# aws-neuron/neuronx-distributed

Measured on AMD Instinct MI355X. Metric: tokens/sec (whole node) Llama-2-7B training, TP=num_gpus, seq=4096, higher is better.
Workload: dtype bf16; 1 GPU; model=llama2-7b, global_batch=32, seq_len=4096, parallelism=tp1, zero1=True

## Files before the change

### neuronx_distributed_amd/models/gpt2.py

```python

from dataclasses import dataclass

import torch
import torch.nn as nn

from ..parallel.layers import (
    ColumnParallelLinear,
    RowParallelLinear,
    ParallelEmbedding,
)
from ..parallel.layer_norm import LayerNorm
from ..parallel.loss_functions import parallel_cross_entropy

torch.fx.wrap("parallel_cross_entropy")
from ..parallel import parallel_state as ps
from ..kernels.flash_attn import flash_attn_func


@dataclass
class GPT2Config:
    hidden_size: int = 768
    num_hidden_layers: int = 12
    num_attention_heads: int = 12
    vocab_size: int = 50304
# ... 48 lines not shown
        qkv = self.c_attn(x)
        q, k, v = qkv.chunk(3, dim=-1)
        q = q.reshape(B, S, self.n_local, self.head_dim).transpose(1, 2)
        k = k.reshape(B, S, self.n_local, self.head_dim).transpose(1, 2)
        v = v.reshape(B, S, self.n_local, self.head_dim).transpose(1, 2)
        if kv_cache is not None:
            k, v = kv_cache.update(k.contiguous(), v.contiguous(), pos_offset)
        out = flash_attn_func(q.contiguous(), k.contiguous(), v.contiguous(),
                              causal=True)
        out = out.transpose(1, 2).reshape(B, S, -1)
        return self.c_proj(out)


class GPT2MLP(nn.Module):
    def __init__(self, cfg: GPT2Config):
        super().__init__()
        self.c_fc = ColumnParallelLinear(
            cfg.hidden_size, 4 * cfg.hidden_size, bias=True,
            gather_output=False, init_method=_init(cfg.initializer_range))
        self.c_proj = RowParallelLinear(
            4 * cfg.hidden_size, cfg.hidden_size, bias=True,
            input_is_parallel=True, init_method=_init(cfg.initializer_range))

    def forward(self, x):
        return self.c_proj(torch.nn.functional.gelu(self.c_fc(x)))


class GPT2Block(nn.Module):
    def __init__(self, cfg: GPT2Config):
        super().__init__()
        self.ln_1 = LayerNorm(cfg.hidden_size, eps=cfg.layer_norm_epsilon)
        self.attn = GPT2Attention(cfg)
        self.ln_2 = LayerNorm(cfg.hidden_size, eps=cfg.layer_norm_epsilon)
        self.mlp = GPT2MLP(cfg)

    def forward(self, x, pos_offset=0, kv_cache=None):
        x = x + self.attn(self.ln_1(x), pos_offset, kv_cache)
        return x + self.mlp(self.ln_2(x))


class GPT2LMHeadModel(nn.Module):
    def __init__(self, cfg: GPT2Config):
        super().__init__()
        self.config = cfg
        self.wte = ParallelEmbedding(cfg.vocab_size, cfg.hidden_size,
                                     init_method=_init(cfg.initializer_range))
        self.wpe = nn.Embedding(cfg.max_position_embeddings, cfg.hidden_size)
        nn.init.normal_(self.wpe.weight, std=cfg.initializer_range)
        self.h = nn.ModuleList(GPT2Block(cfg)
                               for _ in range(cfg.num_hidden_layers))
        self.ln_f = LayerNorm(cfg.hidden_size, eps=cfg.layer_norm_epsilon)
        self.lm_head = ColumnParallelLinear(
            cfg.hidden_size, cfg.vocab_size, bias=False, gather_output=False,
            init_method=_init(cfg.initializer_range))

    def forward(self, input_ids, labels=None, pos_offset=0, kv_caches=None):
        B, S = input_ids.shape
        pos = torch.arange(pos_offset, pos_offset + S,
                           device=input_ids.device)
        x = self.wte(input_ids) + self.wpe(pos)
        for i, block in enumerate(self.h):
            kc = kv_caches[i] if kv_caches is not None else None
            x = block(x, pos_offset, kc)
        x = self.ln_f(x)
        logits = self.lm_head(x)
        if labels is None:
            return logits
        shift = labels[:, 1:].contiguous()
        loss = parallel_cross_entropy(logits[:, :-1, :].contiguous(), shift)
        return loss.sum() / (shift != -100).sum().clamp(min=1)
```

### neuronx_distributed_amd/models/gpt_neox.py

```python

from dataclasses import dataclass

import torch
import torch.nn as nn

from .. import ops
from ..kernels.flash_attn import flash_attn_func
from ..parallel import parallel_state as ps
from ..parallel.layer_norm import LayerNorm
from ..parallel.layers import (
    ColumnParallelLinear,
    ParallelEmbedding,
    RowParallelLinear,
)
from ..parallel.loss_functions import parallel_cross_entropy

torch.fx.wrap("parallel_cross_entropy")


@dataclass
class GPTNeoXConfig:
    hidden_size: int = 6144
    intermediate_size: int = 24576
    num_hidden_layers: int = 44
# ... 83 lines not shown
                              causal=True)
        out = out.transpose(1, 2).reshape(B, S, -1)
        return self.dense(out)


class GPTNeoXMLP(nn.Module):
    def __init__(self, cfg: GPTNeoXConfig):
        super().__init__()
        self.dense_h_to_4h = ColumnParallelLinear(
            cfg.hidden_size, cfg.intermediate_size, bias=True,
            gather_output=False, init_method=_init(cfg.initializer_range))
        self.dense_4h_to_h = RowParallelLinear(
            cfg.intermediate_size, cfg.hidden_size, bias=True,
            input_is_parallel=True, init_method=_init(cfg.initializer_range))

    def forward(self, x):
        return self.dense_4h_to_h(
            torch.nn.functional.gelu(self.dense_h_to_4h(x)))


class GPTNeoXLayer(nn.Module):
    def __init__(self, cfg: GPTNeoXConfig):
        super().__init__()
        self.use_parallel_residual = cfg.use_parallel_residual
        self.input_layernorm = LayerNorm(cfg.hidden_size,
                                         eps=cfg.layer_norm_epsilon)
        self.post_attention_layernorm = LayerNorm(cfg.hidden_size,
                                                  eps=cfg.layer_norm_epsilon)
        self.attention = GPTNeoXAttention(cfg)
        self.mlp = GPTNeoXMLP(cfg)

    def forward(self, x, cos, sin, pos_offset=0, kv_cache=None):
        attn_out = self.attention(self.input_layernorm(x), cos, sin,
                                  pos_offset, kv_cache)
        if self.use_parallel_residual:
            return x + attn_out + self.mlp(self.post_attention_layernorm(x))
        h = x + attn_out
        return h + self.mlp(self.post_attention_layernorm(h))


class GPTNeoXForCausalLM(nn.Module):
    def __init__(self, cfg: GPTNeoXConfig):
        super().__init__()
        self.config = cfg
        self.embed_in = ParallelEmbedding(
            cfg.vocab_size, cfg.hidden_size,
            init_method=_init(cfg.initializer_range))
        self.layers = nn.ModuleList(GPTNeoXLayer(cfg)
                                    for _ in range(cfg.num_hidden_layers))
        self.final_layer_norm = LayerNorm(cfg.hidden_size,
                                          eps=cfg.layer_norm_epsilon)
        self.embed_out = ColumnParallelLinear(
            cfg.hidden_size, cfg.vocab_size, bias=False, gather_output=False,
            init_method=_init(cfg.initializer_range))
        cos, sin = ops.precompute_rope_freqs(
            cfg.max_position_embeddings,
            max(2, 2 * (int(cfg.head_dim * cfg.rotary_pct) // 2)),
            cfg.rope_theta)
        self.register_buffer("rope_cos", cos, persistent=False)
        self.register_buffer("rope_sin", sin, persistent=False)

    def reset_parameters(self):
        cfg = self.config
        cos, sin = ops.precompute_rope_freqs(
            cfg.max_position_embeddings,
            max(2, 2 * (int(cfg.head_dim * cfg.rotary_pct) // 2)),
            cfg.rope_theta, device=self.rope_cos.device)
        with torch.no_grad():
            self.rope_cos.copy_(cos)
            self.rope_sin.copy_(sin)

    def forward(self, input_ids, labels=None, pos_offset=0, kv_caches=None):
        x = self.embed_in(input_ids)
        for i, layer in enumerate(self.layers):
            kc = kv_caches[i] if kv_caches is not None else None
            x = layer(x, self.rope_cos, self.rope_sin, pos_offset, kc)
        x = self.final_layer_norm(x)
        logits = self.embed_out(x)
        if labels is None:
            return logits
        shift = labels[:, 1:].contiguous()
        loss = parallel_cross_entropy(logits[:, :-1, :].contiguous(), shift)
        return loss.sum() / (shift != -100).sum().clamp(min=1)
```

### neuronx_distributed_amd/models/llama.py

```python

import math
import os
from dataclasses import dataclass, field
from typing import Optional

import torch
import torch.nn as nn

from .. import ops
from ..parallel import parallel_state as ps
from ..parallel.layers import (
    ColumnParallelLinear,
    RowParallelLinear,
    ParallelEmbedding,
)
from ..parallel.qkv_linear import GQAQKVColumnParallelLinear
from ..parallel.loss_functions import parallel_cross_entropy

torch.fx.wrap("parallel_cross_entropy")
from ..parallel.mappings import (
    scatter_to_sequence_parallel_region,
    gather_from_sequence_parallel_region,
)
from ..kernels.flash_attn import flash_attn_func
# ... 337 lines not shown
        if (not isinstance(hidden, torch.fx.Proxy)
                and not self.training and not torch.is_grad_enabled()
                and hidden.is_cuda and hidden.dtype == torch.bfloat16
                and not self.config.sequence_parallel_enabled
                and self.config.hidden_size % 8 == 0
                and ops.add_rmsnorm_available()
                and all(hasattr(l, "forward_fused")
                        for l in self.layers)):
            residual, delta = hidden, None
            for i, layer in enumerate(self.layers):
                kc = kv_caches[i] if kv_caches is not None else None
                residual, delta = layer.forward_fused(
                    residual, delta, self.rope_cos, self.rope_sin,
                    pos_offset, kc)
            _, hidden = ops.add_rmsnorm(residual, delta, self.norm.weight,
                                        self.norm.variance_epsilon)
            return hidden
        if fused_norm_train_ok(self.config, hidden, self.training) \
                and kv_caches is None \
                and all(hasattr(l, "forward_fused_train")
                        and not l._forward_hooks
                        and not l._forward_pre_hooks
                        for l in self.layers):
            residual, delta = hidden, None
            for layer in self.layers:
                residual, delta = layer.forward_fused_train(
                    residual, delta, self.rope_cos, self.rope_sin,
                    pos_offset)
            _, hidden = ops.add_rmsnorm_train(delta, residual,
                                              self.norm.weight,
                                              self.norm.variance_epsilon)
        else:
            for i, layer in enumerate(self.layers):
                kc = kv_caches[i] if kv_caches is not None else None
                hidden = layer(hidden, self.rope_cos, self.rope_sin,
                               pos_offset, kc)
            hidden = self.norm(hidden)
        if self.config.sequence_parallel_enabled:
            hidden = gather_from_sequence_parallel_region(
                hidden, seq_dim=0, to_model_parallel=True)
            hidden = hidden.transpose(0, 1)
        return hidden


class LlamaForCausalLM(nn.Module):
    supports_tensor_position = True

    def __init__(self, config: LlamaConfig):
        super().__init__()
        self.config = config
        self.model = LlamaModel(config)
        self.lm_head = ColumnParallelLinear(
            config.hidden_size, config.vocab_size, bias=False,
            gather_output=False,
            init_method=_init_method(config.initializer_range))
        if config.tie_word_embeddings:
            self.lm_head.weight = self.model.embed_tokens.weight

    def forward(self, input_ids, labels=None, pos_offset=0, kv_caches=None):
        hidden = self.model(input_ids, pos_offset, kv_caches)
        if labels is not None and self.config.loss_chunks > 0:
            from ..utils.chunked_loss import chunked_lm_loss

            return chunked_lm_loss(hidden, self.lm_head, labels,
                                   num_chunks=self.config.loss_chunks)
        logits = self.lm_head(hidden)
        if labels is None:
            return logits
        shift = labels[:, 1:].contiguous()
        loss = parallel_cross_entropy(logits[:, :-1, :].contiguous(), shift)
        valid = (shift != -100).sum().clamp(min=1)
        return loss.sum() / valid
```

### neuronx_distributed_amd/models/mixtral.py

```python

from dataclasses import dataclass
from typing import Optional

import os

import torch
import torch.nn as nn

from ..moe.expert_mlps import ExpertMLPs
from ..moe.loss_function import load_balancing_loss_func
from ..moe.model import MoE
from ..moe.routing import (GroupLimitedRouter, RouterSinkhorn, RouterTopK)
from ..moe.shared_experts import SharedExperts
from ..parallel.layers import ColumnParallelLinear, ParallelEmbedding
from ..parallel.loss_functions import parallel_cross_entropy
from ..parallel.mappings import (
    gather_from_sequence_parallel_region,
    scatter_to_sequence_parallel_region,
)
from .. import ops
from .llama import (LlamaAttention, LlamaMLP, RMSNorm, _init_method,
                    fused_norm_train_ok)

torch.fx.wrap("parallel_cross_entropy")
# ... 151 lines not shown
        cos, sin = ops.precompute_rope_freqs(
            self.config.max_position_embeddings, self.config.head_dim,
            self.config.rope_theta, device=self.rope_cos.device)
        with torch.no_grad():
            self.rope_cos.copy_(cos)
            self.rope_sin.copy_(sin)

    def forward(self, input_ids, pos_offset=0, kv_caches=None):
        hidden = self.embed_tokens(input_ids)
        if self.config.sequence_parallel_enabled:
            hidden = hidden.transpose(0, 1).contiguous()
            hidden = scatter_to_sequence_parallel_region(hidden, seq_dim=0)
        all_router_logits = []
        if fused_norm_train_ok(self.config, hidden, self.training) \
                and kv_caches is None \
                and all(hasattr(l, "forward_fused_train")
                        and not l._forward_hooks
                        and not l._forward_pre_hooks
                        for l in self.layers):
            residual, delta = hidden, None
            for layer in self.layers:
                residual, delta, router_logits = layer.forward_fused_train(
                    residual, delta, self.rope_cos, self.rope_sin,
                    pos_offset)
                if router_logits is not None:
                    all_router_logits.append(router_logits)
            _, hidden = ops.add_rmsnorm_train(delta, residual,
                                              self.norm.weight,
                                              self.norm.variance_epsilon)
        else:
            for i, layer in enumerate(self.layers):
                kc = kv_caches[i] if kv_caches is not None else None
                hidden, router_logits = layer(hidden, self.rope_cos,
                                              self.rope_sin, pos_offset, kc)
                if router_logits is not None:
                    all_router_logits.append(router_logits)
            hidden = self.norm(hidden)
        if self.config.sequence_parallel_enabled:
            hidden = gather_from_sequence_parallel_region(
                hidden, seq_dim=0, to_model_parallel=True)
            hidden = hidden.transpose(0, 1)
        return hidden, all_router_logits


class MixtralForCausalLM(nn.Module):
    supports_tensor_position = True

    def __init__(self, config: MixtralConfig):
        super().__init__()
        self.config = config
        self.model = MixtralModel(config)
        self.lm_head = ColumnParallelLinear(
            config.hidden_size, config.vocab_size, bias=False,
            gather_output=False,
            init_method=_init_method(config.initializer_range))
        if config.tie_word_embeddings:
            self.lm_head.weight = self.model.embed_tokens.weight

    def forward(self, input_ids, labels=None, pos_offset=0, kv_caches=None):
        hidden, router_logits = self.model(input_ids, pos_offset, kv_caches)
        logits = self.lm_head(hidden)
        if labels is None:
            return logits
        shift = labels[:, 1:].contiguous()
        loss = parallel_cross_entropy(logits[:, :-1, :].contiguous(),
                                      shift).sum() / \
            (shift != -100).sum().clamp(min=1)
        if router_logits and self.config.router_aux_loss_coef > 0:
            aux = load_balancing_loss_func(
                torch.cat(router_logits, dim=0),
                self.config.num_local_experts,
                self.config.num_experts_per_tok)
            loss = loss + self.config.router_aux_loss_coef * aux
        return loss
```

### neuronx_distributed_amd/ops/__init__.py

```python

import ctypes
import math
import os
from typing import Optional

import torch

_LIB = None
_LIB_ERR = None


def _load():
    global _LIB, _LIB_ERR
    if _LIB is not None or _LIB_ERR is not None:
        return _LIB
    from .build import LIB

    if not os.path.exists(LIB):
        _LIB_ERR = f"{LIB} not built — run neuronx_distributed_amd.ops.build"
        return None
    try:
        lib = ctypes.CDLL(LIB)
    except OSError as e:
        _LIB_ERR = str(e)
# ... 414 lines not shown
            dk = dk_pq
            dv = dv_pq
        return dq, dk, dv, None, None, None


def flash_attn(q, k, v, causal=True, softmax_scale=None, window=0):
    scale = softmax_scale or 1.0 / math.sqrt(q.shape[-1])
    return _FlashAttnFn.apply(q, k, v, causal, scale, window)


def flash_attn_window_available() -> bool:
    lib = _load()
    return lib is not None and hasattr(lib, "flash_attn_fwd_window")


def flash_attn_windowed(q, k, v, window: int, softmax_scale=None):
    lib = _require_lib()
    B, Hq, S, D = q.shape
    Hkv = k.shape[1]
    assert D == 128 and q.dtype == torch.bfloat16
    scale = softmax_scale or 1.0 / math.sqrt(D)
    q, k, v = q.contiguous(), k.contiguous(), v.contiguous()
    out = torch.empty_like(q)
    lse = torch.empty(B, Hq, S, dtype=torch.float32, device=q.device)
    lib.flash_attn_fwd_window(_ptr(q), _ptr(k), _ptr(v), _ptr(out),
                              _ptr(lse), ctypes.c_int(B), ctypes.c_int(Hq),
                              ctypes.c_int(Hkv), ctypes.c_int(S),
                              ctypes.c_float(scale), ctypes.c_int(window),
                              _stream())
    return out



def adamw_step(master: torch.Tensor, m: torch.Tensor, v: torch.Tensor,
               grad_bf16: torch.Tensor, param_bf16: torch.Tensor,
               clip: Optional[torch.Tensor], lr: float, beta1: float,
               beta2: float, eps: float, weight_decay: float, step: int):
    lib = _require_lib()
    n = master.numel()
    assert m.numel() == n and v.numel() == n and grad_bf16.numel() == n
    assert grad_bf16.dtype == torch.bfloat16 and param_bf16.dtype == torch.bfloat16
    inv_bc1 = 1.0 / (1.0 - beta1 ** step)
    inv_bc2 = 1.0 / (1.0 - beta2 ** step)
    lib.adamw_step(ctypes.c_long(n), _ptr(master), _ptr(m), _ptr(v),
                   _ptr(grad_bf16), _ptr(param_bf16),
                   _ptr(clip) if clip is not None else None,
                   ctypes.c_float(lr), ctypes.c_float(beta1),
                   ctypes.c_float(beta2), ctypes.c_float(eps),
                   ctypes.c_float(weight_decay), ctypes.c_float(inv_bc1),
                   ctypes.c_float(inv_bc2), _stream())



_MOE_MB = 16


def moe_decode_available() -> bool:
    lib = _load()
    return lib is not None and hasattr(lib, "moe_decode_glu")


def moe_decode_glu(hidden: torch.Tensor, gate_up_w: torch.Tensor,
                   down_w: torch.Tensor, expert_affinities: torch.Tensor,
                   expert_index: torch.Tensor) -> torch.Tensor:
    lib = _require_lib()
    T, H = hidden.shape
    E, _, twoI = gate_up_w.shape
    I = twoI // 2
    assert H % 64 == 0 and I % 64 == 0, (H, I)
    k = expert_index.shape[1]
    dev = hidden.device

    flat_e = expert_index.reshape(-1)
    order = torch.argsort(flat_e, stable=True)
    sorted_e = flat_e[order].to(torch.long)
    sorted_tok = (order // k).to(torch.int32)

    counts = torch.bincount(flat_e, minlength=E)
    blocks_per_e = (counts + _MOE_MB - 1) // _MOE_MB
    nb = int(blocks_per_e.sum().item())
    if nb == 0:
        return hidden.new_zeros(T, H)
    blockbase = torch.cumsum(torch.nn.functional.pad(blocks_per_e, (1, 0)),
                             0)
    countbase = torch.cumsum(torch.nn.functional.pad(counts, (1, 0)), 0)

    within = torch.arange(T * k, device=dev) - countbase[sorted_e]
    padded_idx = (blockbase[sorted_e] + within // _MOE_MB) * _MOE_MB + \
        within % _MOE_MB

    slot_token = torch.zeros(nb * _MOE_MB, dtype=torch.int32, device=dev)
    slot_token[padded_idx] = sorted_tok
    aff = torch.zeros(nb * _MOE_MB, dtype=torch.float32, device=dev)
    aff[padded_idx] = expert_affinities.float()[
        sorted_tok.long(), sorted_e]

    block_expert = torch.repeat_interleave(
        torch.arange(E, device=dev), blocks_per_e).to(torch.int32)
    bi = torch.arange(nb, device=dev)
    block_ord = bi - blockbase[block_expert.long()]
    block_len = torch.clamp(counts[block_expert.long()] -
                            _MOE_MB * block_ord, 0, _MOE_MB).to(torch.int32)

    act = torch.empty(nb * _MOE_MB, I, dtype=torch.bfloat16, device=dev)
    out = torch.zeros(T, H, dtype=torch.float32, device=dev)
    hidden = hidden.contiguous()
# ... 199 lines not shown
```

### neuronx_distributed_amd/optimizer/zero_redundancy_optimizer.py

```python

import math
import os
from typing import Dict, List

import torch
import torch.distributed as dist

from ..parallel import comm, parallel_state as ps
from ..parallel.utils import param_is_tensor_parallel, param_is_expert_parallel
from ..utils.logger import get_logger

logger = get_logger(__name__)

_DEFAULT_BUCKET_CAP_MB = 130


def _bucket_cap_bytes():
    return int(os.environ.get("ALL_GATHER_REDUCE_SCATTER_BUCKET_CAP_MB",
                              _DEFAULT_BUCKET_CAP_MB)) * 1024 * 1024


class _Bucket:

    def __init__(self, params: List[torch.nn.Parameter], group_info,
                 group_index: int, optimizer_dtype,
                 fp32_grad_acc: bool = False):
        self.params = params
        self.group_info = group_info
        self.group_index = group_index
        self.fp32_grad_acc = fp32_grad_acc
        world = group_info.size
        device = params[0].device
        dtype = params[0].dtype

        numel = sum(p.numel() for p in params)
        self.padded = int(math.ceil(numel / world) * world)
        self.flat_param = torch.zeros(self.padded, dtype=dtype, device=device)
        grad_dtype = torch.float32 if fp32_grad_acc else dtype
        self.flat_grad = torch.zeros(self.padded, dtype=grad_dtype,
                                     device=device)

        self.segments = []
        off = 0
        with torch.no_grad():
            for p in params:
                n = p.numel()
                self.flat_param[off:off + n].copy_(p.data.reshape(-1))
                new_data = self.flat_param[off:off + n].view(p.shape)
                p.data = new_data
                if fp32_grad_acc:
                    seg = self.flat_grad[off:off + n]

                    def _acc(param, _seg=seg):
                        if param.grad is not None:
                            _seg.add_(param.grad.detach().reshape(-1).float())
                            param.grad = None

                    p.register_post_accumulate_grad_hook(_acc)
                else:
                    p.grad = self.flat_grad[off:off + n].view(p.shape)
                self.segments.append((p, off, off + n))
# ... 122 lines not shown
                        cur, ginfo, gi, self.optimizer_dtype,
                        self.use_fp32_grad_acc))


    def _bucket_grad_scale(self, b) -> float:
        ep_size = ps._GROUPS["ep"].size if "ep" in ps._GROUPS else 1
        if ep_size > 1 and b.group_info.name == "edp":
            return 1.0 / (b.group_info.size * ep_size)
        return 1.0 / b.group_info.size

    @torch.no_grad()
    def _reduce_scatter_grads(self):
        works = []
        for b in self.buckets:
            world = b.group_info.size
            scale = self._bucket_grad_scale(b)
            if world == 1:
                if scale != 1.0:
                    b.flat_grad.mul_(scale)
                b.grad_shard = b.flat_grad
                continue
            b.flat_grad.mul_(scale)
            if comm._backend_is_gloo(b.group_info.group):
                dist.all_reduce(b.flat_grad, group=b.group_info.group)
                b.grad_shard.copy_(b.flat_grad[b.shard_lo:b.shard_hi])
            else:
                w = dist.reduce_scatter_tensor(b.grad_shard, b.flat_grad,
                                               group=b.group_info.group,
                                               async_op=True)
                works.append(w)
        for w in works:
            w.wait()

    @torch.no_grad()
    def _clip_grads(self, apply: bool = True):
        device = self.buckets[0].master.device
        sq = torch.zeros(1, dtype=torch.float32, device=device)
        for b in self.buckets:
            sq += b.local_sq_norm()
        comm.all_reduce(sq, group=self._sharding_group)
        for name in ("tp", "pp"):
            if name in ps._GROUPS and ps._GROUPS[name].size > 1:
                comm.all_reduce(sq, group=ps._GROUPS[name])
        total_norm = sq.sqrt()
        self._grad_norm = total_norm.squeeze()
        clip = torch.clamp(self.max_norm / (total_norm + 1e-6), max=1.0)
        if apply:
            for b in self.buckets:
                b.grad_shard.mul_(clip)
        return clip

    @torch.no_grad()
    def _all_gather_params(self, copy_master: bool = True):
        works = []
        for b in self.buckets:
            shard = b.flat_param[b.shard_lo:b.shard_hi]
            if copy_master:
                shard.copy_(b.master.to(b.flat_param.dtype))
            world = b.group_info.size
            if world == 1:
                continue
            if comm._backend_is_gloo(b.group_info.group):
                parts = list(b.flat_param.chunk(world))
                dist.all_gather(parts, shard.clone(), group=b.group_info.group)
            else:
                w = dist.all_gather_into_tensor(b.flat_param, shard.clone(),
                                                group=b.group_info.group,
                                                async_op=True)
                works.append(w)
        for w in works:
            w.wait()

    def _use_fused(self) -> bool:
        from .. import ops

        return (self.use_fused_kernel
                and not self.use_fp32_grad_acc
                and self.optimizer_class is torch.optim.AdamW
                and self.optimizer_dtype == torch.float32
                and self.buckets and self.buckets[0].master.is_cuda
                and ops.is_available())

    @torch.no_grad()
    def _fused_step(self, clip):
        from .. import ops

        self._step_count = getattr(self, "_step_count", 0) + 1
        for b in self.buckets:
            group = self.param_groups[b.group_index]
            if not hasattr(b, "fused_m"):
                b.fused_m = torch.zeros_like(b.master)
                b.fused_v = torch.zeros_like(b.master)
            beta1, beta2 = group.get("betas", (0.9, 0.999))
            ops.adamw_step(b.master, b.fused_m, b.fused_v, b.grad_shard,
                           b.flat_param[b.shard_lo:b.shard_hi], clip,
                           group.get("lr", 1e-3), beta1, beta2,
                           group.get("eps", 1e-8),
                           group.get("weight_decay", 0.0), self._step_count)

    @torch.no_grad()
    def step(self, closure=None):
        loss = None
        if closure is not None:
            with torch.enable_grad():
                loss = closure()

# ... 84 lines not shown
```

### neuronx_distributed_amd/parallel/layers.py

```python

import math
import os
from typing import Callable, Optional

import torch
import torch.nn as nn
import torch.nn.functional as F
import torch.distributed as dist

from . import comm
from . import parallel_state as ps
from .mappings import (
    copy_to_tensor_model_parallel_region,
    gather_from_tensor_model_parallel_region,
    reduce_from_tensor_model_parallel_region,
    reduce_scatter_to_sequence_parallel_region,
    gather_from_sequence_parallel_region,
    scatter_to_tensor_model_parallel_region,
)
from .random import get_rng_state_tracker
from .utils import (
    create_local_weight,
    divide,
    set_tensor_model_parallel_attributes,
# ... 71 lines not shown
                      + (weight.shape[0],),
                      dtype=input_.dtype, device=input_.device)
    for t in range(world):
        owner = (me - t) % world
        works = []
        if t < world - 1:
            ops_ = [dist.P2POp(dist.isend, cur, nxt, group=tp_info.group),
                    dist.P2POp(dist.irecv, recv_buf, prv,
                               group=tp_info.group)]
            works = dist.batch_isend_irecv(ops_)
        out[owner * S:(owner + 1) * S] = F.linear(cur, weight)
        for w in works:
            w.wait()
        if t < world - 1:
            nxt_recv = spare if cur is src else cur
            cur = recv_buf
            recv_buf = nxt_recv
    if bias is not None:
        out = out + bias
    return out


class _RPLOverlappedLinearRS(torch.autograd.Function):

    @staticmethod
    def forward(ctx, input_parallel, weight):
        tp_info = ps.get_group_info("tp")
        world = tp_info.size
        me = tp_info.rank_in_group(dist.get_rank())
        ranks = tp_info.ranks_of(dist.get_rank())
        ctx.save_for_backward(input_parallel, weight)
        x = input_parallel.contiguous()
        assert x.shape[0] % world == 0
        Sc = x.shape[0] // world
        handles = []
        chunks = []
        mine = None
        for c in range(world):
            y = F.linear(x[c * Sc:(c + 1) * Sc], weight)
            chunks.append(y)
            handles.append(dist.reduce(y, dst=ranks[c],
                                       group=tp_info.group, async_op=True))
            if c == me:
                mine = y
        for h in handles:
            h.wait()
        return mine.clone()

    @staticmethod
    def backward(ctx, grad_output):
        input_parallel, weight = ctx.saved_tensors
        tp_info = ps.get_group_info("tp")
        g = comm.all_gather(grad_output.contiguous(), dim=0, group=tp_info)
        grad_input = g.matmul(weight)
        go2d = g.reshape(-1, g.shape[-1])
        in2d = input_parallel.reshape(-1, input_parallel.shape[-1])
        grad_weight = go2d.t().matmul(in2d)
        return grad_input, grad_weight


def _fp8_forward_enabled() -> bool:
    return os.environ.get("NXDA_FP8_LINEAR", "0") == "1"


def _fp8_eligible(x: torch.Tensor, w: torch.Tensor) -> bool:
    return (x.is_cuda and x.dtype == torch.bfloat16
            and w.dtype == torch.bfloat16
            and x.shape[-1] % 16 == 0 and w.shape[0] % 16 == 0
            and w.shape[0] >= 2 * w.shape[1]
            and x.numel() // x.shape[-1] >= 2048)


def _fp8_quantized_weight(weight: torch.Tensor):
    from ..quantization.quantization_config import (QuantizationConfig,
                                                    QuantizedDtype)
    from ..quantization.quantization_utils import quantize_symmetric

    key = (weight.data_ptr(), weight._version)
    cache = getattr(weight, "_fp8_cache", None)
    if cache is None or cache[0] != key:
        cfg = QuantizationConfig(quantized_dtype=QuantizedDtype.F8E4M3,
                                 quantize_activation=True)
        with torch.no_grad():
            qw, ws = quantize_symmetric(weight.detach(), cfg)
        cache = (key, qw, ws)
        weight._fp8_cache = cache
    return cache[1], cache[2]


def _forward_gemm(total_input: torch.Tensor, weight: torch.Tensor, bias):
    if _fp8_forward_enabled() and _fp8_eligible(total_input, weight):
        from ..quantization.quantization_utils import fp8_scaled_linear

        qw, ws = _fp8_quantized_weight(weight)
        with torch.no_grad():
            out = fp8_scaled_linear(total_input, qw, ws, total_input.dtype)
        if bias is not None:
            out = out + bias
        return out
    return F.linear(total_input, weight, bias)


class LinearWithAsyncCommunication(torch.autograd.Function):

    @staticmethod
    def forward(ctx, input_, weight, bias, async_grad_allreduce,
                sequence_parallel_enabled, save_for_backward=True):
        ctx.use_bias = bias is not None
        ctx.async_grad_allreduce = async_grad_allreduce
        ctx.sequence_parallel_enabled = sequence_parallel_enabled
        ctx.compute_weight_gradient = weight.requires_grad

        if sequence_parallel_enabled:
            tp_info = ps.get_group_info("tp")
            if os.environ.get("NXDA_SP_OVERLAP", "0") == "1" and \
                    tp_info.size > 1 and not ps.is_aot_mode():
                output = _sp_overlapped_linear(input_, weight, bias, tp_info)
                if save_for_backward:
                    if ctx.compute_weight_gradient:
                        ctx.save_for_backward(input_, weight)
                    else:
                        ctx.save_for_backward(weight)
                return output
            total_input = comm.all_gather(input_, dim=0, group=tp_info)
        else:
            total_input = input_

        output = _forward_gemm(total_input, weight, bias)

        if save_for_backward:
            if ctx.compute_weight_gradient:
                ctx.save_for_backward(input_, weight)
            else:
                ctx.save_for_backward(weight)
        return output

    @staticmethod
    def backward(ctx, grad_output):
        if ctx.compute_weight_gradient:
            input_, weight = ctx.saved_tensors
        else:
            (weight,) = ctx.saved_tensors
            input_ = None

        tp_info = ps.get_group_info("tp")
        handle = None

        grad_output = grad_output.contiguous()
        grad_input = grad_output.matmul(weight)

        if ctx.sequence_parallel_enabled and ctx.compute_weight_gradient:
            total_input = comm.all_gather(input_, dim=0, group=tp_info)
        else:
            total_input = input_

        if ctx.sequence_parallel_enabled:
            world = tp_info.size
            if world > 1 and not ps.is_aot_mode():
                gi = grad_input.contiguous()
                sub_shape = (gi.shape[0] // world,) + tuple(gi.shape[1:])
                grad_input_out = torch.empty(sub_shape, dtype=gi.dtype,
                                             device=gi.device)
                if comm._backend_is_gloo(tp_info.group):
                    dist.all_reduce(gi, group=tp_info.group)
                    rank = tp_info.rank_in_group(dist.get_rank())
                    grad_input_out.copy_(gi[rank * sub_shape[0]:(rank + 1) * sub_shape[0]])
                else:
                    handle = dist.reduce_scatter_tensor(
                        grad_input_out, gi, group=tp_info.group, async_op=True)
                grad_input = grad_input_out
        elif ctx.async_grad_allreduce:
            handle = comm.all_reduce(grad_input, group=tp_info, async_op=True)

        grad_weight = grad_bias = None
        if ctx.compute_weight_gradient:
            go2d = grad_output.reshape(-1, grad_output.shape[-1])
            in2d = total_input.reshape(-1, total_input.shape[-1])
            grad_weight = go2d.t().matmul(in2d)
            if ctx.use_bias:
                grad_bias = go2d.sum(dim=0)
        elif ctx.use_bias:
            grad_bias = grad_output.reshape(-1, grad_output.shape[-1]).sum(dim=0)

        if handle is not None:
            handle.wait()
        return grad_input, grad_weight, grad_bias, None, None, None


def linear_with_async_allreduce(input_, weight, bias=None,
                                async_grad_allreduce=False,
                                sequence_parallel_enabled=False):
    from .. import ops as _ops

    if _ops.use_skinny_linear(input_, weight, sequence_parallel_enabled):
        flat = input_.reshape(-1, input_.shape[-1]).contiguous()
        out = _ops.skinny_linear(flat, weight)
        if bias is not None:
            out = out + bias
        return out.reshape(*input_.shape[:-1], weight.shape[0])
    args = cast_if_autocast_enabled(input_, weight, bias)
    with torch.amp.autocast("cuda", enabled=False):
        return LinearWithAsyncCommunication.apply(
            *args, async_grad_allreduce, sequence_parallel_enabled)


class BaseParallelLinear(nn.Module):
    def reset_parameters(self):
        spec = getattr(self, "_reset_spec", None)
        if spec is None:
            return
        out_f, in_f, per_part, pdim, stride, init_method, dtype = spec
        _initialize_affine_weight(self.weight, out_f, in_f, per_part,
                                  partition_dim=pdim, init_method=init_method,
                                  stride=stride, dtype=dtype)
        if getattr(self, "bias", None) is not None:
            with torch.no_grad():
                self.bias.zero_()

    def _init_weight(self, weight, init_method):
        if getattr(weight, "device", torch.device("cpu")).type == "meta":
            return
        with get_rng_state_tracker().fork():
            init_method(weight)

    def preshard_hook(self, model_state_dict: dict, prefix: str) -> None:
        name = prefix.rsplit(".", 1)[0] if prefix.endswith("weight") else prefix
        for pname, param in self.named_parameters():
            key = f"{name}.{pname}" if not prefix.endswith(pname) else prefix
            if key not in model_state_dict:
                continue
            full = model_state_dict[key]
            pdim = getattr(param, "partition_dim", -1)
            if pdim < 0 or not getattr(param, "tensor_model_parallel", False):
                continue
            if full.shape[pdim] == param.shape[pdim]:
                continue
            model_state_dict[key] = create_local_weight(
                full, pdim, param.shape[pdim], getattr(param, "partition_stride", 1))


class ColumnParallelLinear(BaseParallelLinear):

    def __init__(self, input_size, output_size, bias=True, gather_output=True,
                 dtype=None, device=None, init_method=None, stride=1,
                 sequence_parallel_enabled=False, keep_master_weight=False,
                 skip_bias_add=False):
        super().__init__()
        self.input_size = input_size
        self.output_size = output_size
        self.gather_output = gather_output
        self.sequence_parallel_enabled = sequence_parallel_enabled
        self.skip_bias_add = skip_bias_add
        self.stride = stride
        world = ps.get_tensor_model_parallel_size()
        self.output_size_per_partition = divide(output_size, world)
        dtype = dtype or torch.get_default_dtype()
        self.dtype = dtype
        init_method = init_method or default_init_method

        self.weight = nn.Parameter(
            torch.empty(self.output_size_per_partition, input_size, dtype=dtype,
                        device=device))
        self._reset_spec = (output_size, input_size,
                            self.output_size_per_partition, 0, stride,
                            init_method, dtype)
        self.master_weight = _initialize_affine_weight(
            self.weight, output_size, input_size, self.output_size_per_partition,
            partition_dim=0, init_method=init_method, stride=stride,
            return_master_weight=keep_master_weight, dtype=dtype)

        if bias:
            self.bias = nn.Parameter(
                torch.zeros(self.output_size_per_partition, dtype=dtype,
                            device=device))
            set_tensor_model_parallel_attributes(self.bias, world > 1, 0, stride,
                                                 world)
        else:
            self.register_parameter("bias", None)

        self.async_tensor_model_parallel_allreduce = (
            not sequence_parallel_enabled and world > 1)

    def forward(self, input_):
        if self.async_tensor_model_parallel_allreduce or self.sequence_parallel_enabled:
            input_parallel = input_
        else:
            input_parallel = copy_to_tensor_model_parallel_region(input_)

        bias = self.bias if not self.skip_bias_add else None
        output_parallel = linear_with_async_allreduce(
            input_parallel, self.weight, bias,
            async_grad_allreduce=self.async_tensor_model_parallel_allreduce,
            sequence_parallel_enabled=self.sequence_parallel_enabled)

        if self.gather_output:
            output = gather_from_tensor_model_parallel_region(output_parallel)
        else:
            output = output_parallel
        if self.skip_bias_add:
            return output, self.bias
        return output


class RowParallelLinear(BaseParallelLinear):

    def __init__(self, input_size, output_size, bias=True,
                 input_is_parallel=True, dtype=None, device=None,
                 init_method=None, stride=1, sequence_parallel_enabled=False,
                 keep_master_weight=False, skip_bias_add=False,
                 reduce_output=True):
        super().__init__()
        self.input_size = input_size
        self.output_size = output_size
        self.input_is_parallel = input_is_parallel
        self.sequence_parallel_enabled = sequence_parallel_enabled
        self.skip_bias_add = skip_bias_add
        self.reduce_output = reduce_output
        world = ps.get_tensor_model_parallel_size()
        self.input_size_per_partition = divide(input_size, world)
        dtype = dtype or torch.get_default_dtype()
        self.dtype = dtype
        init_method = init_method or default_init_method

        self.weight = nn.Parameter(
            torch.empty(output_size, self.input_size_per_partition, dtype=dtype,
                        device=device))
        self._reset_spec = (output_size, input_size,
                            self.input_size_per_partition, 1, stride,
                            init_method, dtype)
        self.master_weight = _initialize_affine_weight(
            self.weight, output_size, input_size, self.input_size_per_partition,
            partition_dim=1, init_method=init_method, stride=stride,
            return_master_weight=keep_master_weight, dtype=dtype)

        if bias:
            self.bias = nn.Parameter(torch.zeros(output_size, dtype=dtype,
                                                 device=device))
        else:
            self.register_parameter("bias", None)

    def forward(self, input_):
        if self.input_is_parallel:
# ... 125 lines not shown
```

### neuronx_distributed_amd/parallel/qkv_linear.py

```python

from typing import Optional

import torch
import torch.nn as nn
import torch.nn.functional as F
import torch.distributed as dist

from . import comm
from . import parallel_state as ps
from .layers import BaseParallelLinear, default_init_method
from .utils import divide, set_tensor_model_parallel_attributes


def _sp_overlapped_qkv(input_, wq, wk, wv, bq, bk, bv, tp_info):
    import torch.distributed as dist

    world = tp_info.size
    me = tp_info.rank_in_group(dist.get_rank())
    ranks = tp_info.ranks_of(dist.get_rank())
    nxt = ranks[(me + 1) % world]
    prv = ranks[(me - 1) % world]
    S = input_.shape[0]
    src = input_.contiguous()
    cur = src
    recv_buf = torch.empty_like(src)
    spare = torch.empty_like(src)
    lead = tuple(input_.shape[1:-1])
    q = torch.empty((world * S,) + lead + (wq.shape[0],),
                    dtype=input_.dtype, device=input_.device)
    k = torch.empty((world * S,) + lead + (wk.shape[0],),
                    dtype=input_.dtype, device=input_.device)
    v = torch.empty((world * S,) + lead + (wv.shape[0],),
                    dtype=input_.dtype, device=input_.device)
    for t in range(world):
        owner = (me - t) % world
        works = []
        if t < world - 1:
            ops_ = [dist.P2POp(dist.isend, cur, nxt, group=tp_info.group),
                    dist.P2POp(dist.irecv, recv_buf, prv,
                               group=tp_info.group)]
            works = dist.batch_isend_irecv(ops_)
        sl = slice(owner * S, (owner + 1) * S)
        q[sl] = F.linear(cur, wq, bq)
        k[sl] = F.linear(cur, wk, bk)
        v[sl] = F.linear(cur, wv, bv)
        for w in works:
            w.wait()
        if t < world - 1:
            nxt_recv = spare if cur is src else cur
            cur = recv_buf
            recv_buf = nxt_recv
    return q, k, v


class _QKVLinearWithAsyncCommunication(torch.autograd.Function):
    @staticmethod
    def forward(ctx, input_, wq, wk, wv, bq, bk, bv, sequence_parallel, kv_mult):
        import os

        ctx.sequence_parallel = sequence_parallel
        ctx.kv_mult = kv_mult
        ctx.use_bias = bq is not None
        tp_info = ps.get_group_info("tp")
        if sequence_parallel and tp_info.size > 1 and \
                os.environ.get("NXDA_SP_OVERLAP", "0") == "1" and \
                not ps.is_aot_mode():
            q, k, v = _sp_overlapped_qkv(input_, wq, wk, wv, bq, bk, bv,
                                         tp_info)
            ctx.save_for_backward(input_, wq, wk, wv)
            return q, k, v
        if sequence_parallel:
            total_input = comm.all_gather(input_, dim=0, group=tp_info)
        else:
            total_input = input_
        q = F.linear(total_input, wq, bq)
        k = F.linear(total_input, wk, bk)
        v = F.linear(total_input, wv, bv)
        ctx.save_for_backward(input_, wq, wk, wv)
        return q, k, v

    @staticmethod
    def backward(ctx, gq, gk, gv):
        input_, wq, wk, wv = ctx.saved_tensors
        tp_info = ps.get_group_info("tp")
        world = tp_info.size

        gq = gq.contiguous()
        gk = gk.contiguous()
        gv = gv.contiguous()
        grad_input = gq.matmul(wq)
        grad_input += gk.matmul(wk)
        grad_input += gv.matmul(wv)

        handle = None
        if ctx.sequence_parallel:
            total_input = comm.all_gather(input_, dim=0, group=tp_info)
            if world > 1 and not ps.is_aot_mode():
                sub = (grad_input.shape[0] // world,) + tuple(grad_input.shape[1:])
                gi_out = torch.empty(sub, dtype=grad_input.dtype,
                                     device=grad_input.device)
                if comm._backend_is_gloo(tp_info.group):
                    dist.all_reduce(grad_input, group=tp_info.group)
                    r = tp_info.rank_in_group(dist.get_rank())
                    gi_out.copy_(grad_input[r * sub[0]:(r + 1) * sub[0]])
                else:
                    handle = dist.reduce_scatter_tensor(
                        gi_out, grad_input, group=tp_info.group, async_op=True)
                grad_input = gi_out
        else:
            total_input = input_
            if world > 1:
                handle = comm.all_reduce(grad_input, group=tp_info, async_op=True)

        in2d = total_input.reshape(-1, total_input.shape[-1])
        gq2 = gq.reshape(-1, gq.shape[-1])
        gk2 = gk.reshape(-1, gk.shape[-1])
        gv2 = gv.reshape(-1, gv.shape[-1])
        gwq = gq2.t().matmul(in2d)
        gwk = gk2.t().matmul(in2d)
        gwv = gv2.t().matmul(in2d)
        gbq = gq2.sum(0) if ctx.use_bias else None
        gbk = gk2.sum(0) if ctx.use_bias else None
        gbv = gv2.sum(0) if ctx.use_bias else None

        if handle is not None:
            handle.wait()
        return grad_input, gwq, gwk, gwv, gbq, gbk, gbv, None, None


class GQAQKVColumnParallelLinear(BaseParallelLinear):
    def __init__(self, input_size, output_sizes, bias=False, gather_output=False,
                 dtype=None, device=None, init_method=None,
                 sequence_parallel_enabled=False, kv_size_multiplier=1,
                 num_attention_heads: Optional[int] = None,
                 num_key_value_heads: Optional[int] = None,
                 head_dim: Optional[int] = None):
        super().__init__()
        world = ps.get_tensor_model_parallel_size()
        dtype = dtype or torch.get_default_dtype()
        self.dtype = dtype
        init_method = init_method or default_init_method
        self.sequence_parallel_enabled = sequence_parallel_enabled
        self.gather_output = gather_output
        assert not gather_output, "GQA QKV is used with gather_output=False"

# ... 58 lines not shown

    def _kv_local_rows(self, master: torch.Tensor) -> torch.Tensor:
        world = ps.get_tensor_model_parallel_size()
        rank = ps.get_tensor_model_parallel_rank()
        kvh_rep = self.num_key_value_heads * self.kv_size_multiplier
        per_rank = kvh_rep // world
        rows = []
        for s in range(rank * per_rank, (rank + 1) * per_rank):
            h = s // self.kv_size_multiplier
            rows.append(master[h * self.head_dim:(h + 1) * self.head_dim])
        return torch.cat(rows, dim=0)

    def _deterministic_init(self, input_size, q_out, kv_out, init_method):
        if self.weight_q.device.type == "meta":
            return
        import os

        if os.environ.get("NXDA_FAST_INIT", "0") == "1":
            with torch.no_grad():
                for w in (self.weight_q, self.weight_k, self.weight_v):
                    tmp = torch.empty(w.shape, dtype=torch.float32,
                                      device=w.device)
                    init_method(tmp)
                    w.data.copy_(tmp.to(self.dtype))
            return
        world = ps.get_tensor_model_parallel_size()
        rank = ps.get_tensor_model_parallel_rank()
        with torch.no_grad():
            mq = torch.empty(q_out, input_size, dtype=torch.float32, device="cpu")
            init_method(mq)
            rows = self.q_output_size_per_partition
            self.weight_q.data.copy_(mq[rank * rows:(rank + 1) * rows].to(self.dtype))
            for name, w in (("k", self.weight_k), ("v", self.weight_v)):
                m = torch.empty(kv_out, input_size, dtype=torch.float32, device="cpu")
                init_method(m)
                w.data.copy_(self._kv_local_rows(m).to(self.dtype))

    def preshard_hook(self, model_state_dict: dict, prefix: str) -> None:
        base = prefix.rsplit(".", 1)[0]
        world = ps.get_tensor_model_parallel_size()
        rank = ps.get_tensor_model_parallel_rank()
        for pname in ("weight_q", "bias_q"):
            key = f"{base}.{pname}"
            if key in model_state_dict:
                full = model_state_dict[key]
                rows = full.shape[0] // world
                model_state_dict[key] = full[rank * rows:(rank + 1) * rows]
        for pname in ("weight_k", "weight_v", "bias_k", "bias_v"):
            key = f"{base}.{pname}"
            if key in model_state_dict:
                model_state_dict[key] = self._kv_local_rows(model_state_dict[key])

    def _fused_qkv_weight(self):
        key = tuple((w._version, w.data_ptr())
                    for w in (self.weight_q, self.weight_k, self.weight_v))
        cached = getattr(self, "_qkv_cat_cache", None)
        if cached is None or cached[0] != key:
            with torch.no_grad():
                wcat = torch.cat([self.weight_q.detach(),
                                  self.weight_k.detach(),
                                  self.weight_v.detach()], dim=0).contiguous()
                bcat = None
                if self.bias_q is not None:
                    bcat = torch.cat([self.bias_q.detach(),
                                      self.bias_k.detach(),
                                      self.bias_v.detach()]).contiguous()
            cached = (key, wcat, bcat)
            self._qkv_cat_cache = cached
        return cached[1], cached[2]

    def forward(self, input_):
        from .. import ops as _ops

        if (not torch.is_grad_enabled() and not self.training
                and not isinstance(input_, torch.fx.Proxy) and input_.is_cuda
                and not self.sequence_parallel_enabled
                and not ps.is_aot_mode()):
            wcat, bcat = self._fused_qkv_weight()
            out = F.linear(input_, wcat, bcat)
            nq = self.q_output_size_per_partition
            nkv = self.kv_output_size_per_partition
            q = out[..., :nq]
            k = out[..., nq:nq + nkv]
            v = out[..., nq + nkv:]
            return q, k, v
        if _ops.use_skinny_linear(input_, self.weight_q,
                                  self.sequence_parallel_enabled) and \
                self.bias_q is None:
            flat = input_.reshape(-1, input_.shape[-1]).contiguous()
            lead = input_.shape[:-1]
            q = _ops.skinny_linear(flat, self.weight_q)
            k = _ops.skinny_linear(flat, self.weight_k)
            v = _ops.skinny_linear(flat, self.weight_v)
            return (q.reshape(*lead, -1), k.reshape(*lead, -1),
                    v.reshape(*lead, -1))
        q, k, v = _QKVLinearWithAsyncCommunication.apply(
            input_, self.weight_q, self.weight_k, self.weight_v,
            self.bias_q, self.bias_k, self.bias_v,
            self.sequence_parallel_enabled, self.kv_size_multiplier)
        return q, k, v


def allreduce_kv_shared_gradients(parameters):
    if "kv" not in ps._GROUPS:
        return
    grads = [p.grad for p in parameters
             if p.grad is not None and getattr(p, "kv_shared", False)]
# ... 7 lines not shown
```

### neuronx_distributed_amd/utils/medusa_utils.py

```python

from typing import List

import torch


def generate_medusa_buffers(medusa_choices: List[List[int]], device=None):
    sorted_choices = sorted(medusa_choices, key=lambda p: (len(p), p))
    n = len(sorted_choices) + 1

    attn_mask = torch.eye(n, dtype=torch.bool)
    attn_mask[:, 0] = True
    paths = {(): 0}
    for i, path in enumerate(sorted_choices):
        paths[tuple(path)] = i + 1
        for d in range(1, len(path)):
            anc = paths[tuple(path[:d])]
            attn_mask[i + 1, anc] = True

    position_ids = torch.tensor([0] + [len(p) for p in sorted_choices])

    max_k = max((p[-1] for p in sorted_choices), default=0) + 1
    tree_indices = torch.zeros(n, dtype=torch.long)
    for i, path in enumerate(sorted_choices):
        tree_indices[i + 1] = (len(path) - 1) * max_k + path[-1] + 1

    leaves = [p for p in sorted_choices
              if not any(len(q) == len(p) + 1 and q[:len(p)] == list(p)
                         for q in sorted_choices)]
    depth = max((len(p) for p in sorted_choices), default=0)
    retrieve = torch.full((len(leaves), depth + 1), -1, dtype=torch.long)
    for li, leaf in enumerate(leaves):
        retrieve[li, 0] = 0
        for d in range(1, len(leaf) + 1):
            retrieve[li, d] = paths[tuple(leaf[:d])]

    out = {
        "medusa_attn_mask": attn_mask,
        "tree_indices": tree_indices,
        "medusa_position_ids": position_ids,
        "retrieve_indices": retrieve,
    }
    if device is not None:
        out = {k: v.to(device) for k, v in out.items()}
    return out


class MedusaHead(torch.nn.Module):

    def __init__(self, hidden_size: int, vocab_size: int, dtype=None):
        super().__init__()
        from ..parallel.layers import ColumnParallelLinear

        self.proj = torch.nn.Linear(hidden_size, hidden_size, dtype=dtype)
        self.act = torch.nn.SiLU()
        self.lm_head = ColumnParallelLinear(hidden_size, vocab_size,
                                            bias=False, gather_output=False,
                                            dtype=dtype)

    def forward(self, hidden):
        return self.lm_head(hidden + self.act(self.proj(hidden)))
```

Baseline: 24320 tokens/s.

## Transpose weights with custom HIP kernel for backward dgrad GEMMs

Adds a tiled bf16 transpose HIP kernel (single and batched) and uses it in backward passes to materialise a transposed copy of large weights. The input-gradient GEMM then runs as F.linear against that copy instead of matmul with the original weight. The aim is to give the BLAS library a preferred operand layout for dgrad, at the cost of an extra weight-sized transpose per layer per backward. It also introduces a global weight generation counter, bumped by ZeRO all-gather, for cache keys, and opts LM heads out of the shadow path.

```diff
diff --git a/neuronx_distributed_amd/models/gpt2.py b/neuronx_distributed_amd/models/gpt2.py
--- a/neuronx_distributed_amd/models/gpt2.py
+++ b/neuronx_distributed_amd/models/gpt2.py
@@ -124,7 +124,7 @@
         self.ln_f = LayerNorm(cfg.hidden_size, eps=cfg.layer_norm_epsilon)
         self.lm_head = ColumnParallelLinear(
             cfg.hidden_size, cfg.vocab_size, bias=False, gather_output=False,
-            init_method=_init(cfg.initializer_range))
+            dgrad_shadow=False, init_method=_init(cfg.initializer_range))
 
     def forward(self, input_ids, labels=None, pos_offset=0, kv_caches=None):
         B, S = input_ids.shape
diff --git a/neuronx_distributed_amd/models/gpt_neox.py b/neuronx_distributed_amd/models/gpt_neox.py
--- a/neuronx_distributed_amd/models/gpt_neox.py
+++ b/neuronx_distributed_amd/models/gpt_neox.py
@@ -159,7 +159,7 @@
                                           eps=cfg.layer_norm_epsilon)
         self.embed_out = ColumnParallelLinear(
             cfg.hidden_size, cfg.vocab_size, bias=False, gather_output=False,
-            init_method=_init(cfg.initializer_range))
+            dgrad_shadow=False, init_method=_init(cfg.initializer_range))
         cos, sin = ops.precompute_rope_freqs(
             cfg.max_position_embeddings,
             max(2, 2 * (int(cfg.head_dim * cfg.rotary_pct) // 2)),
diff --git a/neuronx_distributed_amd/models/llama.py b/neuronx_distributed_amd/models/llama.py
--- a/neuronx_distributed_amd/models/llama.py
+++ b/neuronx_distributed_amd/models/llama.py
@@ -413,7 +413,7 @@
         self.model = LlamaModel(config)
         self.lm_head = ColumnParallelLinear(
             config.hidden_size, config.vocab_size, bias=False,
-            gather_output=False,
+            gather_output=False, dgrad_shadow=False,
             init_method=_init_method(config.initializer_range))
         if config.tie_word_embeddings:
             self.lm_head.weight = self.model.embed_tokens.weight
diff --git a/neuronx_distributed_amd/models/mixtral.py b/neuronx_distributed_amd/models/mixtral.py
--- a/neuronx_distributed_amd/models/mixtral.py
+++ b/neuronx_distributed_amd/models/mixtral.py
@@ -227,7 +227,7 @@
         self.model = MixtralModel(config)
         self.lm_head = ColumnParallelLinear(
             config.hidden_size, config.vocab_size, bias=False,
-            gather_output=False,
+            gather_output=False, dgrad_shadow=False,
             init_method=_init_method(config.initializer_range))
         if config.tie_word_embeddings:
             self.lm_head.weight = self.model.embed_tokens.weight
diff --git a/neuronx_distributed_amd/ops/__init__.py b/neuronx_distributed_amd/ops/__init__.py
--- a/neuronx_distributed_amd/ops/__init__.py
+++ b/neuronx_distributed_amd/ops/__init__.py
@@ -490,6 +490,87 @@
 
 
 
+def transpose_available() -> bool:
+    lib = _load()
+    return lib is not None and hasattr(lib, "transpose_bf16")
+
+
+def _transpose_tiles(lib, who: str, x: torch.Tensor, out: torch.Tensor):
+    if x.dim() != 2 or x.dtype != torch.bfloat16 or not x.is_cuda:
+        raise ValueError(f"{who}: source must be a 2-D bf16 GPU tensor, got "
+                         f"{tuple(x.shape)} {x.dtype} on {x.device}")
+    R, C = x.shape
+    rs = x.stride(0) if R > 1 else max(C, 8)
+    if x.stride(1) != 1 and C > 1:
+        raise ValueError(f"{who}: source rows must be dense, strides "
+                         f"{x.stride()}")
+    if out.dtype != x.dtype or out.device != x.device or \
+            tuple(out.shape) != (C, R) or not out.is_contiguous():
+        raise ValueError(f"{who}: destination must be a contiguous "
+                         f"{(C, R)} bf16 tensor on {x.device}, got "
+                         f"{tuple(out.shape)} strides {out.stride()}")
+    lib.transpose_bf16_tiles.restype = ctypes.c_long
+    tiles = lib.transpose_bf16_tiles(ctypes.c_long(R), ctypes.c_long(C),
+                                     ctypes.c_long(rs))
+    if tiles < 0 or x.data_ptr() % 16 or out.data_ptr() % 16:
+        raise ValueError(f"{who}: shape {(R, C)} row stride {rs} outside the "
+                         f"kernel contract (R, C, stride multiples of 8, "
+                         f"16-byte aligned)")
+    return tiles, rs
+
+
+def transpose(x: torch.Tensor, out: Optional[torch.Tensor] = None):
+    if x.dim() != 2:
+        raise ValueError(f"transpose: 2-D input expected, got {tuple(x.shape)}")
+    if out is None:
+        out = torch.empty(x.shape[1], x.shape[0], dtype=x.dtype,
+                          device=x.device)
+    if not x.is_cuda:
+        out.copy_(x.t())
+        return out
+    lib = _require_lib()
+    _, rs = _transpose_tiles(lib, "transpose", x, out)
+    rc = lib.transpose_bf16(_ptr(x), _ptr(out), ctypes.c_long(rs),
+                            ctypes.c_long(x.shape[0]),
+                            ctypes.c_long(x.shape[1]), _stream())
+    if rc != 0:
+        raise ValueError(f"transpose rejected shape {tuple(x.shape)}")
+    return out
+
+
+def transpose_batched(xs, outs=None):
+    xs = list(xs)
+    if outs is None:
+        outs = [torch.empty(x.shape[1], x.shape[0], dtype=x.dtype,
+                            device=x.device) for x in xs]
+    outs = list(outs)
+    if len(outs) != len(xs):
+        raise ValueError("transpose_batched: one destination per source")
+    if not xs:
+        return outs
+    if not xs[0].is_cuda:
+        for x, o in zip(xs, outs):
+            transpose(x, o)
+        return outs
+    lib = _require_lib()
+    rows, first = [], 0
+    for x, o in zip(xs, outs):
+        if x.device != xs[0].device:
+            raise ValueError("transpose_batched: all sources on one device")
+        tiles, rs = _transpose_tiles(lib, "transpose_batched", x, o)
+        rows.append([x.data_ptr(), o.data_ptr(), rs, x.shape[0], x.shape[1],
+                     first])
+        first += tiles
+    desc = torch.tensor(rows, dtype=torch.int64).to(xs[0].device)
+    rc = lib.transpose_bf16_batched(_ptr(desc), len(rows),
+                                    ctypes.c_long(first), _stream())
+    if rc != 0:
+        raise ValueError(f"transpose_batched rejected {len(rows)} matrices, "
+                         f"{first} tiles")
+    return outs
+
+
+
 _MOE_MB = 16
 
 
diff --git a/neuronx_distributed_amd/ops/csrc/transpose.hip b/neuronx_distributed_amd/ops/csrc/transpose.hip
--- /dev/null
+++ b/neuronx_distributed_amd/ops/csrc/transpose.hip
@@ -0,0 +1,95 @@
+
+#include "common.h"
+
+typedef unsigned u4v __attribute__((ext_vector_type(4)));
+
+#define TR_TILE 64
+
+__device__ __forceinline__ void transpose_tile(
+    const short* __restrict__ src, short* __restrict__ dst, long src_stride,
+    int R, int C, int tr, int tc, unsigned* tile) {
+  const int t = threadIdx.x;
+  const int ch = t & 7, rp = t >> 3;
+  const int r0 = tr * TR_TILE, c0 = tc * TR_TILE;
+  {
+    const int r = r0 + 2 * rp, c = c0 + 8 * ch;
+    if (r < R && c < C) {
+      const short* p = src + (long)r * src_stride + c;
+      u4v a = *(const u4v*)p;
+      u4v b = *(const u4v*)(p + src_stride);
+      unsigned* w = tile + (8 * ch) * 32 + (rp ^ (ch << 2));
+#pragma unroll
+      for (int k = 0; k < 4; ++k) {
+        w[(2 * k) * 32] = (a[k] & 0xffffu) | (b[k] << 16);
+        w[(2 * k + 1) * 32] = (a[k] >> 16) | (b[k] & 0xffff0000u);
+      }
+    }
+  }
+  __syncthreads();
+#pragma unroll
+  for (int it = 0; it < 2; ++it) {
+    const int cl = it * 32 + (t >> 3), q = t & 7;
+    const int c = c0 + cl, r = r0 + 8 * q;
+    if (c < C && r < R) {
+      u4v v = *(const u4v*)(tile + cl * 32 + ((q ^ ((cl >> 3) & 7)) << 2));
+      *(u4v*)(dst + (long)c * R + r) = v;
+    }
+  }
+}
+
+extern "C" __global__ void __launch_bounds__(256)
+transpose_bf16_kernel(const short* __restrict__ src, short* __restrict__ dst,
+                      long src_stride, int R, int C, int tiles_c) {
+  __shared__ __attribute__((aligned(16))) unsigned tile[TR_TILE * 32];
+  const int b = blockIdx.x;
+  transpose_tile(src, dst, src_stride, R, C, b / tiles_c, b % tiles_c, tile);
+}
+
+#define TR_DESC 6
+
+extern "C" __global__ void __launch_bounds__(256)
+transpose_bf16_batched_kernel(const long* __restrict__ desc, int n) {
+  __shared__ __attribute__((aligned(16))) unsigned tile[TR_TILE * 32];
+  const int b = blockIdx.x;
+  int lo = 0, hi = n - 1;
+  while (lo < hi) {
+    int mid = (lo + hi + 1) >> 1;
+    if (desc[(long)mid * TR_DESC + 5] <= b) lo = mid; else hi = mid - 1;
+  }
+  const long* d = desc + (long)lo * TR_DESC;
+  const int R = (int)d[3], C = (int)d[4];
+  const int tiles_c = (C + TR_TILE - 1) / TR_TILE;
+  const int local = b - (int)d[5];
+  transpose_tile((const short*)d[0], (short*)d[1], d[2], R, C,
+                 local / tiles_c, local % tiles_c, tile);
+}
+
+static inline long transpose_tiles(long R, long C) {
+  return ((R + TR_TILE - 1) / TR_TILE) * ((C + TR_TILE - 1) / TR_TILE);
+}
+
+extern "C" long transpose_bf16_tiles(long R, long C, long src_stride) {
+  if (R <= 0 || C <= 0 || (R & 7) || (C & 7) || (src_stride & 7) ||
+      src_stride < C || R > 0x7fffffffL || C > 0x7fffffffL)
+    return -1;
+  long tiles = transpose_tiles(R, C);
+  return tiles > 0x7fffffffL ? -1 : tiles;
+}
+
+extern "C" int transpose_bf16(const void* src, void* dst, long src_stride,
+                              long R, long C, hipStream_t stream) {
+  long tiles = transpose_bf16_tiles(R, C, src_stride);
+  if (tiles < 0 || ((uintptr_t)src & 15) || ((uintptr_t)dst & 15)) return 1;
+  transpose_bf16_kernel<<<(unsigned)tiles, 256, 0, stream>>>(
+      (const short*)src, (short*)dst, src_stride, (int)R, (int)C,
+      (int)((C + TR_TILE - 1) / TR_TILE));
+  return 0;
+}
+
+extern "C" int transpose_bf16_batched(const void* desc, int n,
+                                      long total_tiles, hipStream_t stream) {
+  if (n <= 0 || total_tiles <= 0 || total_tiles > 0x7fffffffL) return 1;
+  transpose_bf16_batched_kernel<<<(unsigned)total_tiles, 256, 0, stream>>>(
+      (const long*)desc, n);
+  return 0;
+}
diff --git a/neuronx_distributed_amd/optimizer/zero_redundancy_optimizer.py b/neuronx_distributed_amd/optimizer/zero_redundancy_optimizer.py
--- a/neuronx_distributed_amd/optimizer/zero_redundancy_optimizer.py
+++ b/neuronx_distributed_amd/optimizer/zero_redundancy_optimizer.py
@@ -7,6 +7,7 @@
 import torch.distributed as dist
 
 from ..parallel import comm, parallel_state as ps
+from ..parallel.layers import bump_weight_generation
 from ..parallel.utils import param_is_tensor_parallel, param_is_expert_parallel
 from ..utils.logger import get_logger
 
@@ -235,6 +236,7 @@
 
     @torch.no_grad()
     def _all_gather_params(self, copy_master: bool = True):
+        bump_weight_generation()
         works = []
         for b in self.buckets:
             shard = b.flat_param[b.shard_lo:b.shard_hi]
diff --git a/neuronx_distributed_amd/parallel/layers.py b/neuronx_distributed_amd/parallel/layers.py
--- a/neuronx_distributed_amd/parallel/layers.py
+++ b/neuronx_distributed_amd/parallel/layers.py
@@ -147,7 +147,7 @@
         input_parallel, weight = ctx.saved_tensors
         tp_info = ps.get_group_info("tp")
         g = comm.all_gather(grad_output.contiguous(), dim=0, group=tp_info)
-        grad_input = g.matmul(weight)
+        grad_input = _dgrad(g, weight)
         go2d = g.reshape(-1, g.shape[-1])
         in2d = input_parallel.reshape(-1, input_parallel.shape[-1])
         grad_weight = go2d.t().matmul(in2d)
@@ -166,12 +166,28 @@
             and x.numel() // x.shape[-1] >= 2048)
 
 
+_WEIGHT_GENERATION = [0]
+
+
+def bump_weight_generation() -> int:
+    _WEIGHT_GENERATION[0] += 1
+    return _WEIGHT_GENERATION[0]
+
+
+def weight_generation() -> int:
+    return _WEIGHT_GENERATION[0]
+
+
+def _weight_cache_key(weight: torch.Tensor):
+    return (weight.data_ptr(), weight._version, _WEIGHT_GENERATION[0])
+
+
 def _fp8_quantized_weight(weight: torch.Tensor):
     from ..quantization.quantization_config import (QuantizationConfig,
                                                     QuantizedDtype)
     from ..quantization.quantization_utils import quantize_symmetric
 
-    key = (weight.data_ptr(), weight._version)
+    key = _weight_cache_key(weight)
     cache = getattr(weight, "_fp8_cache", None)
     if cache is None or cache[0] != key:
         cfg = QuantizationConfig(quantized_dtype=QuantizedDtype.F8E4M3,
@@ -194,6 +210,38 @@
             out = out + bias
         return out
     return F.linear(total_input, weight, bias)
+
+
+def _dgrad_shadow_enabled() -> bool:
+    return os.environ.get("NXDA_DGRAD_SHADOW", "1") == "1"
+
+
+_DGRAD_SHADOW_MIN_NUMEL = 4096 * 4096
+
+
+def _dgrad_shadow_eligible(weight: torch.Tensor) -> bool:
+    return (weight.dim() == 2 and weight.dtype == torch.bfloat16
+            and weight.is_contiguous()
+            and weight.numel() >= _DGRAD_SHADOW_MIN_NUMEL
+            and weight.shape[0] % 8 == 0 and weight.shape[1] % 8 == 0
+            and getattr(weight, "dgrad_shadow", True))
+
+
+def dgrad_weight_t(weight: torch.Tensor) -> Optional[torch.Tensor]:
+    if torch.is_grad_enabled():
+        return None
+    if not (_dgrad_shadow_enabled() and _dgrad_shadow_eligible(weight)):
+        return None
+    from .. import ops as _ops
+
+    return _ops.transpose(weight.detach())
+
+
+def _dgrad(grad_output: torch.Tensor, weight: torch.Tensor) -> torch.Tensor:
+    w_t = dgrad_weight_t(weight)
+    if w_t is None:
+        return grad_output.matmul(weight)
+    return F.linear(grad_output, w_t)
 
 
 class LinearWithAsyncCommunication(torch.autograd.Function):
@@ -242,7 +290,7 @@
         handle = None
 
         grad_output = grad_output.contiguous()
-        grad_input = grad_output.matmul(weight)
+        grad_input = _dgrad(grad_output, weight)
 
         if ctx.sequence_parallel_enabled and ctx.compute_weight_gradient:
             total_input = comm.all_gather(input_, dim=0, group=tp_info)
@@ -339,11 +387,12 @@
     def __init__(self, input_size, output_size, bias=True, gather_output=True,
                  dtype=None, device=None, init_method=None, stride=1,
                  sequence_parallel_enabled=False, keep_master_weight=False,
-                 skip_bias_add=False):
+                 skip_bias_add=False, dgrad_shadow=True):
         super().__init__()
         self.input_size = input_size
         self.output_size = output_size
         self.gather_output = gather_output
+        self.dgrad_shadow = dgrad_shadow
         self.sequence_parallel_enabled = sequence_parallel_enabled
         self.skip_bias_add = skip_bias_add
         self.stride = stride
@@ -383,6 +432,8 @@
             input_parallel = copy_to_tensor_model_parallel_region(input_)
 
         bias = self.bias if not self.skip_bias_add else None
+        if not self.dgrad_shadow:
+            self.weight.dgrad_shadow = False
         output_parallel = linear_with_async_allreduce(
             input_parallel, self.weight, bias,
             async_grad_allreduce=self.async_tensor_model_parallel_allreduce,
diff --git a/neuronx_distributed_amd/parallel/qkv_linear.py b/neuronx_distributed_amd/parallel/qkv_linear.py
--- a/neuronx_distributed_amd/parallel/qkv_linear.py
+++ b/neuronx_distributed_amd/parallel/qkv_linear.py
@@ -8,7 +8,8 @@
 
 from . import comm
 from . import parallel_state as ps
-from .layers import BaseParallelLinear, default_init_method
+from .layers import (BaseParallelLinear, default_init_method, _dgrad,
+                     _weight_cache_key, dgrad_weight_t)
 from .utils import divide, set_tensor_model_parallel_attributes
 
 
@@ -88,9 +89,14 @@
         gq = gq.contiguous()
         gk = gk.contiguous()
         gv = gv.contiguous()
-        grad_input = gq.matmul(wq)
-        grad_input += gk.matmul(wk)
-        grad_input += gv.matmul(wv)
+        grad_input = _dgrad(gq, wq)
+        for g, w in ((gk, wk), (gv, wv)):
+            w_t = dgrad_weight_t(w)
+            if w_t is None:
+                grad_input += g.matmul(w)
+            else:
+                gi2d = grad_input.view(-1, grad_input.shape[-1])
+                torch.addmm(gi2d, g.view(-1, g.shape[-1]), w_t.t(), out=gi2d)
 
         handle = None
         if ctx.sequence_parallel:
@@ -255,7 +261,7 @@
                 model_state_dict[key] = self._kv_local_rows(model_state_dict[key])
 
     def _fused_qkv_weight(self):
-        key = tuple((w._version, w.data_ptr())
+        key = tuple(_weight_cache_key(w)
                     for w in (self.weight_q, self.weight_k, self.weight_v))
         cached = getattr(self, "_qkv_cat_cache", None)
         if cached is None or cached[0] != key:
diff --git a/neuronx_distributed_amd/utils/medusa_utils.py b/neuronx_distributed_amd/utils/medusa_utils.py
--- a/neuronx_distributed_amd/utils/medusa_utils.py
+++ b/neuronx_distributed_amd/utils/medusa_utils.py
@@ -55,7 +55,7 @@
         self.act = torch.nn.SiLU()
         self.lm_head = ColumnParallelLinear(hidden_size, vocab_size,
                                             bias=False, gather_output=False,
-                                            dtype=dtype)
+                                            dtype=dtype, dgrad_shadow=False)
 
     def forward(self, hidden):
         return self.lm_head(hidden + self.act(self.proj(hidden)))
```

Measured after the change: 25110 tokens/s, median of 6. 1.03x the previous value.
